# b41sh/pa

Measured on AMD Instinct MI355X. Metric: decoded GB/s (uncompressed) per node at 1/2/4/8 GPUs; bit-exact vs CPU, higher is better.
Workload: dtype int32

## Files before the change

### pa_amd/csrc/sb_decode.hip

```cpp
#include <hip/hip_runtime.h>
#include <stdint.h>

#include <algorithm>
#include <cstdlib>
#include <map>
#include <mutex>
#include <type_traits>

#include "sb_internal.h"

namespace sbk {

using namespace sb;

#ifndef SB_BLOCK
#define SB_BLOCK 256
#endif
#ifndef SB_LOAD_NT
#define SB_LOAD_NT 1
#endif
#ifndef SB_STORE_NT
#define SB_STORE_NT 1
#endif
#ifndef SB_LDS_DMA
// ... 3861 lines not shown
          run_leaf<1>(s, sh, rs, [&](uint32_t row, const uint32_t* v, uint32_t nv) {
            uint32_t nib = 0;
            for (uint32_t l = 0; l < nv; l++) nib |= (v[l] != 0 ? 1u : 0u) << l;
            if (nib) atomicOr(&xbits[row >> 5], nib << (row & 31));
          });
          __syncthreads();
          if (!sh.err) write_validity(xs, 0, n, pd.row_off, (uint32_t*)a.out_values);
          break;
        }
        case 1:
        case 3: {
          if (tid < 64) {
            const uint32_t r = expand_to_lds(st.codec, a.chunk + pd.byte_off + st.body, st.csize, (lds_u8*)xbits,
                                             (n + 7) / 8);
            if (r) set_err(sh, r);
          }
          __syncthreads();
          if (!sh.err) write_validity(xs, 0, n, pd.row_off, (uint32_t*)a.out_values);
          break;
        }
        case 2:
          if (!Z || need + xb + kZTablesBytes + kStagePad > a.stage_bytes) {
            if (tid == 0) set_err(sh, ST_NYI);
            break;
          }
          if constexpr (Z) if (tid < 64) {
            const uint32_t r = zs::zstd_to_lds(LdsSrc{s.w, s.base + st.body}, st.csize, (lds_u8*)xbits, (n + 7) / 8,
                                               (lds_u8*)xbits + xb, a.stage_bytes - need - xb - kStagePad);
            if (r) set_err(sh, r);
          }
          __syncthreads();
          if (!sh.err) write_validity(xs, 0, n, pd.row_off, (uint32_t*)a.out_values);
          break;
        default:
          if (tid == 0) set_err(sh, ST_OUT_OF_SPEC);
      }
    }
    __syncthreads();
    if (tid == 0) a.status[page] = sh.err;
    __syncthreads();
  }
}

constexpr uint32_t kLvK = 32;
constexpr uint32_t kMaxRuns = 64;

struct LvRuns {
  uint32_t n;
  uint32_t start[kMaxRuns + 1];
  uint32_t arg[kMaxRuns];
};

struct ListShared {
  uint32_t rows, vpos, bw_def, region, fast;
  LvRuns rep, def;
};

__device__ __forceinline__ void put_err(uint32_t* err, uint32_t code) { *err = max(*err, code); }

template <class Src>
__device__ bool parse_runs(const Src& s, uint32_t* err, uint32_t p, uint32_t end, uint32_t L, uint32_t bw, LvRuns& R) {
  uint32_t covered = 0, n = 0;
  while (covered < L) {
    uint32_t h = 0, sft = 0;
    for (;;) {
      if (p >= end || sft > 28) { put_err(err, ST_OUT_OF_SPEC); return false; }
      const uint32_t c = s.u8(p++);
      h |= (c & 0x7Fu) << sft;
      if (!(c & 0x80)) break;
      sft += 7;
    }
    if (n == kMaxRuns) { put_err(err, ST_NYI); return false; }
    R.start[n] = covered;
    if (h & 1) {
      const uint64_t want = (uint64_t)(h >> 1) * bw;
      const uint32_t have = (uint32_t)min<uint64_t>(want, end - p);
      const uint32_t vals = (uint32_t)min<uint64_t>((uint64_t)(h >> 1) * 8, (uint64_t)have * 8 / bw);
      if (vals == 0) { put_err(err, ST_OUT_OF_SPEC); return false; }
      R.arg[n] = 0x80000000u | p;
      p += have;
      covered += vals;
    } else {
      const uint32_t vb = (bw + 7) / 8;
      if (p + vb > end) { put_err(err, ST_OUT_OF_SPEC); return false; }
      uint32_t v = 0;
      for (uint32_t k = 0; k < vb; k++) v |= s.u8(p + k) << (8 * k);
      R.arg[n] = v;
      p += vb;
      covered += h >> 1;
    }
    n++;
  }
  R.start[n] = covered;
  R.n = n;
  return true;
}

template <class Src>
__device__ __forceinline__ uint32_t level_at(const Src& s, const LvRuns& R, uint32_t i, uint32_t bw) {
  uint32_t r = 0;
  if (R.n > 1) {
    uint32_t lo = 0, hi = R.n;
    while (hi - lo > 1) {
      const uint32_t mid = (lo + hi) >> 1;
      if (R.start[mid] <= i) lo = mid; else hi = mid;
    }
    r = lo;
  }
  const uint32_t a = R.arg[r];
  if (!(a & 0x80000000u)) return a;
  const uint32_t bit = (i - R.start[r]) * bw;
  return (s.u32((a & 0x7FFFFFFFu) + (bit >> 3)) >> (bit & 7)) & ((1u << bw) - 1);
}

struct ListArgs {
  const uint8_t* chunk;
  const PageDesc* pages;
  uint32_t n_pages;
  uint32_t nl, ni, ow;
  uint32_t width;
  uint32_t peek;
  uint64_t* counts;
  uint64_t* local;
  uint64_t* blk;
  uint64_t* totals;
  uint4* lvdesc;
  PageDesc* vpages;
  uint8_t* out_offsets;
  uint32_t* out_list_validity;
  uint32_t* out_leaf_validity;
  uint32_t* status;
  uint32_t epoch;
};

template <class Src>
__device__ bool list_parse(const Src& s, uint32_t* err, ListShared& ls, const PageDesc& pd, const ListArgs& a) {
  const uint32_t len = pd.byte_len, L = pd.num_values;
  if (len < 12) { put_err(err, ST_IO); return false; }
  const uint32_t rows = s.u32(0), rl = s.u32(4), dl = s.u32(8);
  if ((uint64_t)12 + rl + dl > len) { put_err(err, ST_IO); return false; }
  const uint32_t max_def = a.nl + 1 + a.ni;
  ls.rows = rows;
  ls.vpos = 12 + rl + dl;
  ls.region = 12 + rl + dl;
  ls.bw_def = 32 - __clz(max_def);
  if (!parse_runs(s, err, 12, 12 + rl, L, 1, ls.rep)) return false;
  if (!parse_runs(s, err, 12 + rl, 12 + rl + dl, L, ls.bw_def, ls.def)) return false;
  if (L > 0 && rows == 0) { put_err(err, ST_OUT_OF_SPEC); return false; }
  ls.fast = ls.rep.n == 1 && (ls.rep.arg[0] & 0x80000000u) && ls.def.n == 1 && (ls.def.arg[0] & 0x80000000u) &&
            ls.bw_def <= 2;
  return true;
}

__device__ __forceinline__ uint32_t compact_even(uint64_t x) {
  x &= 0x5555555555555555ull;
  x = (x | (x >> 1)) & 0x3333333333333333ull;
  x = (x | (x >> 2)) & 0x0F0F0F0F0F0F0F0Full;
  x = (x | (x >> 4)) & 0x00FF00FF00FF00FFull;
  x = (x | (x >> 8)) & 0x0000FFFF0000FFFFull;
  x = (x | (x >> 16)) & 0x00000000FFFFFFFFull;
  return (uint32_t)x;
}

template <class Src>
__device__ __forceinline__ uint64_t ld_bytes(const Src& s, uint32_t p, uint32_t nb, uint32_t end) {
  if (p + 8 <= end) return s.u64(p) & (nb >= 8 ? ~0ull : ((1ull << (8 * nb)) - 1));
  uint64_t v = 0;
  for (uint32_t k = 0; k < nb && p + k < end; k++) v |= (uint64_t)s.u8(p + k) << (8 * k);
  return v;
}

struct LvMasks {
  uint32_t vm, rsm, lfm, lvm, fvm;
};

template <class Src>
__device__ __forceinline__ LvMasks fast_level_masks(const Src& s, uint32_t rp, uint32_t dp, uint32_t region, uint32_t bw,
                                                    uint32_t i0, uint32_t L, uint32_t cs1) {
  LvMasks m{0, 0, 0, 0, 0};
  if (i0 >= L) return m;
  m.vm = L - i0 >= 32 ? 0xFFFFFFFFu : ((1u << (L - i0)) - 1);
  const uint32_t repw = (uint32_t)ld_bytes(s, rp + i0 / 8, 4, dp);
  m.rsm = ~repw & m.vm;
  const uint64_t dw = ld_bytes(s, dp + i0 * bw / 8, 4 * bw, region);
  auto ge = [&](uint32_t t) -> uint32_t {
    if (t == 0) return 0xFFFFFFFFu;
    if (bw == 1) return t == 1 ? (uint32_t)dw : 0u;
    const uint32_t lo = compact_even(dw), hi = compact_even(dw >> 1);
    return t == 1 ? (lo | hi) : t == 2 ? hi : (hi & lo);
  };
  m.lfm = ge(cs1) & m.vm;
  m.lvm = ge(1) & m.vm;
  m.fvm = ge(cs1 + 1) & m.vm;
  return m;
}

template <class Src>
__device__ __forceinline__ LvMasks level_masks(const Src& s, const ListShared& ls, uint32_t i0, uint32_t L,
                                               uint32_t cs1) {
  if (ls.fast)
    return fast_level_masks(s, ls.rep.arg[0] & 0x7FFFFFFFu, ls.def.arg[0] & 0x7FFFFFFFu, ls.region, ls.bw_def, i0, L, cs1);
  LvMasks m{0, 0, 0, 0, 0};
  if (i0 >= L) return m;
  m.vm = L - i0 >= 32 ? 0xFFFFFFFFu : ((1u << (L - i0)) - 1);
  const uint32_t bw = ls.bw_def;
  for (uint32_t k = 0; k < 32; k++) {
    const uint32_t i = i0 + k;
    if (i >= L) break;
    const uint32_t r = level_at(s, ls.rep, i, 1), d = level_at(s, ls.def, i, bw);
    if (r == 0) m.rsm |= 1u << k;
    if (r <= 1 && d >= cs1) m.lfm |= 1u << k;
    if (d > 0) m.lvm |= 1u << k;
    if (d > cs1) m.fvm |= 1u << k;
  }
  return m;
}

__device__ __forceinline__ void lds_or_bits(uint32_t* bm, uint32_t pos, uint64_t v, uint32_t nbits) {
  if (!nbits || !v) return;
  const uint32_t w = pos >> 5, sft = pos & 31;
  const uint64_t lo = v << sft;
  atomicOr(&bm[w], (uint32_t)lo);
  if ((uint32_t)(lo >> 32)) atomicOr(&bm[w + 1], (uint32_t)(lo >> 32));
}

__device__ __forceinline__ void wave_sync() {
  __builtin_amdgcn_fence(__ATOMIC_ACQ_REL, "wavefront");
  __builtin_amdgcn_wave_barrier();
}


__device__ __forceinline__ void wave_put_bits(const uint32_t* bm, uint32_t n, uint64_t g0, uint32_t* out) {
  if (n == 0) return;
  const uint32_t sh = (uint32_t)(g0 & 31), nw = (sh + n + 31) >> 5, eb = (sh + n) & 31;
  uint32_t* o = out + (g0 >> 5);
  for (uint32_t i = threadIdx.x & 63; i < nw; i += 64) {
    const uint32_t v = sh ? __builtin_amdgcn_alignbit(bm[i], bm[(int)i - 1], 32 - sh) : bm[i];
    const bool lo_edge = i == 0 && sh, hi_edge = i == nw - 1 && eb;
    if (lo_edge || hi_edge) {
      uint32_t m = lo_edge ? ~0u << sh : ~0u;
      if (hi_edge) m &= (1u << eb) - 1;
      atomicAnd(&o[i], ~m);
      if (v) atomicOr(&o[i], v);
    } else {
      o[i] = v;
    }
  }
}

#ifndef SB_LV_STAGE
#define SB_LV_STAGE 4160
#endif
#ifndef SB_LV_STAGE_PAD
#define SB_LV_STAGE_PAD 16
#endif
constexpr uint32_t kLvStage = SB_LV_STAGE;
constexpr uint32_t kLvStep = 64 * kLvK;

#ifndef SB_LV_ACC_BITS
#define SB_LV_ACC_BITS 8192
#endif
constexpr uint32_t kLvAccBits = SB_LV_ACC_BITS;
constexpr uint32_t kLvBitsW = kLvAccBits / 32 + 2;

struct ListWave {
  ListShared ls;
  uint32_t err;
  alignas(16) uint16_t obuf[kLvStep + 8];
  uint32_t lbits[kLvBitsW];
  uint32_t fbits[kLvBitsW];
};

struct LvAcc {
  uint32_t r, l;
  uint64_t g0, v0;
};

struct StageSrc {
  LdsSrc l;
  GlbSrc g;
  uint32_t lim;
  __device__ __forceinline__ uint32_t u8(uint32_t i) const { return i < lim ? l.u8(i) : g.u8(i); }
  __device__ __forceinline__ uint32_t u32(uint32_t i) const { return i + 4 <= lim ? l.u32(i) : g.u32(i); }
  __device__ __forceinline__ uint64_t u64(uint32_t i) const { return i + 8 <= lim ? l.u64(i) : g.u64(i); }
};

__device__ __forceinline__ uint32_t compress32(uint32_t x, uint32_t m) {
  x &= m;
  uint32_t mk = ~m << 1;
#pragma unroll
  for (int i = 0; i < 5; i++) {
    uint32_t mp = mk ^ (mk << 1);
    mp ^= mp << 2;
    mp ^= mp << 4;
    mp ^= mp << 8;
    mp ^= mp << 16;
    const uint32_t mv = mp & m;
    m = (m ^ mv) | (mv >> (1 << i));
    const uint32_t t = x & mv;
    x = (x ^ t) | (t >> (1 << i));
    mk &= ~mp;
  }
  return x;
}

__device__ __forceinline__ void lv_flush(ListWave& w, const ListArgs& a, LvAcc& acc) {
  const uint32_t lane = threadIdx.x & 63;
#ifndef SB_V_LV_NOBITS
  if (a.nl) wave_put_bits(w.lbits + 1, acc.r, acc.g0, a.out_list_validity);
  if (a.ni) wave_put_bits(w.fbits + 1, acc.l, acc.v0, a.out_leaf_validity);
#endif
  wave_sync();
  const uint32_t nw = (max(acc.r, acc.l) + 31) / 32 + 2;
  for (uint32_t i = lane; i < nw; i += 64) w.lbits[i] = w.fbits[i] = 0;
  wave_sync();
  acc.g0 += acc.r;
  acc.v0 += acc.l;
  acc.r = acc.l = 0;
}

template <bool WRITE, class WV>
__device__ uint32_t lv_step_m(const LvMasks m, WV& w, uint32_t rows, const ListArgs& a, uint32_t t0, uint64_t rbase,
                              uint64_t lbase, uint32_t carry_r, uint32_t carry_l, uint32_t* step_r, uint32_t* step_l,
                              LvAcc& acc) {
  const uint32_t lane = threadIdx.x & 63;
  if (t0 == 0 && lane == 0 && !(m.rsm & 1)) put_err(&w.err, ST_OUT_OF_SPEC);
  const uint32_t pk = ((uint32_t)__popc(m.rsm) << 16) | (uint32_t)__popc(m.lfm);
  const uint32_t incl = wave_incl_scan(pk), tot = __builtin_amdgcn_readlane(incl, 63), ex = incl - pk;
  const uint32_t rb = carry_r + (ex >> 16), lb = carry_l + (ex & 0xFFFFu);
  uint32_t cm = m.vm;
  if (rb + __popc(m.rsm) > rows) {
    if (rb >= rows + 1) cm = 0;
    else {
      uint32_t x = m.rsm;
      for (uint32_t k = rows - rb; k; k--) x &= x - 1;
      cm = (x & (0u - x)) - 1;
    }
  }
  const uint32_t rsm = m.rsm & cm, lfm = m.lfm & cm;
  if constexpr (WRITE) {
    const uint32_t s_r0 = carry_r, s_l0 = carry_l;
    const uint64_t g0 = rbase + s_r0, v0 = lbase + s_l0;
    const uint32_t al = a.ow == 4 ? (uint32_t)(g0 & 3) : (uint32_t)(g0 & 1);
    if (acc.r + (tot >> 16) > kLvAccBits || acc.l + (tot & 0xFFFFu) > kLvAccBits) lv_flush(w, a, acc);
    const uint32_t pr = acc.r + rb - s_r0, pf = acc.l + lb - s_l0;
    const uint32_t nr = __popc(rsm), nf = __popc(lfm);
    uint16_t* ob = w.obuf + al + (rb - s_r0);
    const uint32_t lrel = lb - s_l0;
    uint32_t j = 0;
#ifndef SB_V_LV_NOOB
    for (uint32_t x = rsm; x; x &= x - 1, j++) ob[j] = (uint16_t)(lrel + __popc(m.lfm & ((x & (0u - x)) - 1)));
#endif
    if (a.nl) lds_or_bits(w.lbits + 1, pr, compress32(m.lvm, rsm), nr);
    if (a.ni) lds_or_bits(w.fbits + 1, pf, compress32(m.fvm, lfm), nf);
    const uint32_t cpk = (nr << 16) | nf;
    const uint32_t ctot = __builtin_amdgcn_readlane(wave_incl_scan(cpk), 63);
    const uint32_t tr = ctot >> 16, tl = ctot & 0xFFFFu;
    wave_sync();
#ifdef SB_V_LV_NOOFF
    constexpr bool wr_off = false;
#else
    constexpr bool wr_off = true;
#endif
    if (!wr_off) {
    } else if (a.ow == 4) {
      uint32_t* o = (uint32_t*)a.out_offsets + (g0 - al);
      const uint32_t v32 = (uint32_t)v0, nq = (al + tr + 3) >> 2;
      for (uint32_t q = lane; q < nq; q += 64) {
        const uint32_t* pr = (const uint32_t*)(w.obuf + 4 * q);
        const uint32_t px = pr[0], py = pr[1];
        const uint32_t e0 = v32 + (px & 0xFFFFu), e1 = v32 + (px >> 16), e2 = v32 + (py & 0xFFFFu), e3 = v32 + (py >> 16);
        const uint32_t j0 = 4 * q;
        if (j0 >= al && j0 + 4 <= al + tr) {
          st_out((u32x4*)(o + j0), u32x4{e0, e1, e2, e3});
        } else {
          const uint32_t e[4] = {e0, e1, e2, e3};
#pragma unroll
          for (uint32_t k = 0; k < 4; k++)
            if (j0 + k >= al && j0 + k < al + tr) o[j0 + k] = e[k];
        }
      }
    } else {
      uint64_t* o = (uint64_t*)a.out_offsets + (g0 - al);
      const uint32_t nq = (al + tr + 1) >> 1;
      for (uint32_t q = lane; q < nq; q += 64) {
        const uint32_t j0 = 2 * q;
        const uint64_t x0 = v0 + w.obuf[j0], x1 = v0 + w.obuf[j0 + 1];
        if (j0 >= al && j0 + 2 <= al + tr) {
          st_out((u32x4*)(o + j0), u32x4{(uint32_t)x0, (uint32_t)(x0 >> 32), (uint32_t)x1, (uint32_t)(x1 >> 32)});
        } else {
          if (j0 >= al && j0 < al + tr) o[j0] = x0;
          if (j0 + 1 >= al && j0 + 1 < al + tr) o[j0 + 1] = x1;
        }
      }
    }
    acc.r += tr;
    acc.l += tl;
    wave_sync();
  }
  *step_r = tot >> 16;
  *step_l = tot & 0xFFFFu;
  return __builtin_amdgcn_readlane(wave_incl_scan(__popc(lfm)), 63);
}

template <bool WRITE, class Src>
__device__ __forceinline__ uint32_t lv_step(const Src& s, ListWave& w, const ListShared& ls, const ListArgs& a,
                                            uint32_t t0, uint32_t L, uint64_t rbase, uint64_t lbase, uint32_t carry_r,
                                            uint32_t carry_l, uint32_t* step_r, uint32_t* step_l, LvAcc& acc) {
  const LvMasks m = level_masks(s, ls, t0 + (threadIdx.x & 63) * kLvK, L, a.nl + 1);
  return lv_step_m<WRITE>(m, w, ls.rows, a, t0, rbase, lbase, carry_r, carry_l, step_r, step_l, acc);
}

template <bool WRITE, class Src>
__device__ void wave_levels(const Src& s, ListWave& w, const ListArgs& a, uint32_t L, uint64_t rbase, uint64_t lbase,
                            uint32_t* rows_c, uint32_t* leaves_c) {
  const uint32_t lane = threadIdx.x & 63, rows = w.ls.rows;
  uint32_t carry_r = 0, carry_l = 0, leaves = 0;
  LvAcc acc{0, 0, rbase, lbase};
  if constexpr (WRITE) {
    for (uint32_t i = lane; i < kLvBitsW; i += 64) w.lbits[i] = w.fbits[i] = 0;
    wave_sync();
  }
  for (uint32_t t0 = 0; t0 < L; t0 += kLvStep) {
    uint32_t sr, sl;
    leaves += lv_step<WRITE>(s, w, w.ls, a, t0, L, rbase, lbase, carry_r, carry_l, &sr, &sl, acc);
    carry_r += sr;
    carry_l += sl;
    if (carry_r > rows) break;
  }
  if constexpr (WRITE) lv_flush(w, a, acc);
  const uint32_t rc = min(carry_r, rows);
  if (lane == 0 && rc != rows) put_err(&w.err, ST_OUT_OF_SPEC);
  *rows_c = rc;
  *leaves_c = leaves;
}

template <class Src>
__device__ __forceinline__ uint32_t lv_count(const Src& s, const ListShared& ls, uint32_t t0, uint32_t L, uint32_t cs1) {
  const LvMasks m = level_masks(s, ls, t0 + (threadIdx.x & 63) * kLvK, L, cs1);
  const uint32_t pk = ((uint32_t)__popc(m.rsm) << 16) | (uint32_t)__popc(m.lfm);
  return __builtin_amdgcn_readlane(wave_incl_scan(pk), 63);
}

__device__ bool wave_page_setup(ListWave& w, uint32_t* stage, const ListArgs& a, uint32_t page, const PageDesc& pd, bool reuse,
                                bool* staged, uint32_t* mis_out, uint32_t* lim_out) {
  const uint32_t lane = threadIdx.x & 63;
  const uint8_t* pg = a.chunk + pd.byte_off;
  const uintptr_t a0 = (uintptr_t)pg & ~(uintptr_t)3;
  const uint32_t mis = (uint32_t)((uintptr_t)pg & 3);
  const uint32_t lim = stage ? min(pd.byte_len, kLvStage) : 0u;
  const uint32_t ndw = (mis + lim + 3) >> 2;
  uint4 d0 = make_uint4(0, 0, 0, 0), d1 = d0;
  if (reuse) {
    d0 = a.lvdesc[2 * page];
    d1 = a.lvdesc[2 * page + 1];
  }
  if (stage) {
    typedef const __attribute__((address_space(1))) uint32_t g32;
    constexpr uint32_t kIt = (kLvStage / 4 + 2 + 63) / 64;
    uint32_t v[kIt];
#pragma unroll
    for (uint32_t k = 0; k < kIt; k++) {
      const uint32_t d = lane + 64 * k;
      v[k] = d < ndw ? __builtin_nontemporal_load((g32*)a0 + d) : 0u;
    }
#pragma unroll
    for (uint32_t k = 0; k < kIt; k++)
      if (lane + 64 * k < ndw) stage[lane + 64 * k] = v[k];
  }
  if (lane == 0) w.err = 0;
  wave_sync();
  *mis_out = mis;
  *lim_out = lim;
  if (reuse && (d0.w & 1)) {
    if (lane == 0) {
      w.ls.rows = d0.x;
      w.ls.vpos = d0.y;
      w.ls.region = d0.y;
      w.ls.bw_def = d0.w >> 1;
      w.ls.fast = 1;
      w.ls.rep.n = w.ls.def.n = 1;
      w.ls.rep.start[0] = w.ls.def.start[0] = 0;
      w.ls.rep.arg[0] = 0x80000000u | d0.z;
      w.ls.def.arg[0] = 0x80000000u | d1.x;
    }
  } else if (lane == 0) {
    const StageSrc ss{LdsSrc{stage, mis}, GlbSrc{pg}, lim};
    list_parse(ss, &w.err, w.ls, pd, a);
  }
  wave_sync();
  if (w.err) return false;
  *staged = w.ls.region <= lim;
  return true;
}

__global__ __launch_bounds__(NT) void k_list_size(ListArgs a) {
  __shared__ ListWave waves[NW];
  __shared__ uint32_t stages[NW][kLvStage / 4 + SB_LV_STAGE_PAD];
  const uint32_t lane = threadIdx.x & 63;
  ListWave& w = waves[threadIdx.x >> 6];
  uint32_t* stage = stages[threadIdx.x >> 6];
  for (uint32_t page = blockIdx.x * NW + (threadIdx.x >> 6); page < a.n_pages; page += gridDim.x * NW) {
    const PageDesc pd = a.pages[page];
    bool staged = false;
    uint32_t mis = 0, lim = 0, rows_c = 0, leaves_c = 0;
    if (wave_page_setup(w, stage, a, page, pd, false, &staged, &mis, &lim)) {
      if (staged) wave_levels<false>(LdsSrc{stage, mis}, w, a, pd.num_values, 0, 0, &rows_c, &leaves_c);
      else wave_levels<false>(GlbSrc{a.chunk + pd.byte_off}, w, a, pd.num_values, 0, 0, &rows_c, &leaves_c);
    }
    wave_sync();
    if (lane == 0) {
      const bool ok = w.err == 0;
      a.counts[page] = ok ? (((uint64_t)rows_c << 32) | leaves_c) : 0;
      const uint32_t fast = ok && w.ls.fast;
      a.lvdesc[2 * page] = make_uint4(w.ls.rows, w.ls.vpos, w.ls.rep.arg[0] & 0x7FFFFFFFu, fast | (w.ls.bw_def << 1));
      a.lvdesc[2 * page + 1] = make_uint4(w.ls.def.arg[0] & 0x7FFFFFFFu, ok, 0, 0);
      a.status[page] = w.err;
    }
    wave_sync();
  }
}

__global__ __launch_bounds__(NT) void k_list_bscan(ListArgs a) {
  __shared__ Shared sh;
  const uint32_t p = blockIdx.x * NT + threadIdx.x;
  uint64_t c = 0;
  if (p < a.n_pages) {
    if (a.peek) {
      const PageDesc pd = a.pages[p];
      const GlbSrc g{a.chunk + pd.byte_off};
      if (pd.byte_len >= 12) {
        const uint64_t vpos = 12ull + g.u32(4) + g.u32(8);
        if (vpos + 9 <= pd.byte_len) c = ((uint64_t)g.u32(0) << 32) | (g.u32((uint32_t)vpos + 5) / a.width);
      }
      a.counts[p] = c;
    } else {
      c = a.counts[p];
    }
  }
  uint64_t tr, tl;
  const uint64_t er = block_excl_scan<uint64_t>(c >> 32, sh, &tr);
  const uint64_t el = block_excl_scan<uint64_t>(c & 0xFFFFFFFFull, sh, &tl);
  if (p < a.n_pages) {
    a.local[2 * p] = er;
    a.local[2 * p + 1] = el;
  }
  if (threadIdx.x == 0) {
    a.blk[2 * blockIdx.x] = tr;
    a.blk[2 * blockIdx.x + 1] = tl;
  }
}

__global__ __launch_bounds__(NT) void k_list_bases(ListArgs a) {
  __shared__ Shared sh;
  __shared__ uint64_t red[2][NW];
  const uint32_t tid = threadIdx.x, lane = tid & 63, wv = tid >> 6;
  const uint32_t p = blockIdx.x * NT + tid;
  uint64_t c = 0;
  uint64_t vpos = ~0ull;
  PageDesc pd{};
  if (p < a.n_pages) {
    if (a.peek) {
      pd = a.pages[p];
      const GlbSrc g{a.chunk + pd.byte_off};
      if (pd.byte_len >= 12) {
        vpos = 12ull + g.u32(4) + g.u32(8);
        if (vpos + 9 <= pd.byte_len) c = ((uint64_t)g.u32(0) << 32) | (g.u32((uint32_t)vpos + 5) / a.width);
      }
      a.counts[p] = c;
    } else {
      c = a.counts[p];
    }
  }
  uint64_t tr, tl;
  const uint64_t er = block_excl_scan<uint64_t>(c >> 32, sh, &tr);
  const uint64_t el = block_excl_scan<uint64_t>(c & 0xFFFFFFFFull, sh, &tl);
  constexpr uint64_t kVal = (1ull << 48) - 1;
  const uint64_t tag = (uint64_t)a.epoch << 48;
  if (tid == 0) {
    __hip_atomic_store(&a.blk[2 * blockIdx.x], tag | tr, __ATOMIC_RELAXED, __HIP_MEMORY_SCOPE_AGENT);
    __hip_atomic_store(&a.blk[2 * blockIdx.x + 1], tag | tl, __ATOMIC_RELAXED, __HIP_MEMORY_SCOPE_AGENT);
  }
  if (wv == 0) {
    uint64_t br = 0, bl = 0;
    for (uint32_t b0 = 0; b0 < blockIdx.x; b0 += 64) {
      const uint32_t b = b0 + lane;
      const bool need = b < blockIdx.x;
      uint64_t r = 0, l = 0;
      for (;;) {
        if (need) {
          r = __hip_atomic_load(&a.blk[2 * b], __ATOMIC_RELAXED, __HIP_MEMORY_SCOPE_AGENT);
          l = __hip_atomic_load(&a.blk[2 * b + 1], __ATOMIC_RELAXED, __HIP_MEMORY_SCOPE_AGENT);
        }
        if (!__ballot(need && ((r & ~kVal) != tag || (l & ~kVal) != tag))) break;
        __builtin_amdgcn_s_sleep(1);
      }
      if (need) {
        br += r & kVal;
        bl += l & kVal;
      }
    }
    br = wave_sum64(br);
    bl = wave_sum64(bl);
    if (lane == 0) {
      red[0][0] = br;
      red[1][0] = bl;
    }
  }
  __syncthreads();
  if (p < a.n_pages) {
    const uint64_t rbase = red[0][0] + er, lbase = red[1][0] + el;
    a.local[2 * p] = rbase;
    a.local[2 * p + 1] = lbase;
    if (p == a.n_pages - 1) {
      const uint64_t tr_all = rbase + (c >> 32), tl_all = lbase + (c & 0xFFFFFFFFull);
      if (a.nl && a.out_list_validity && (tr_all & 31)) a.out_list_validity[tr_all >> 5] = 0;
      if (a.ni && a.out_leaf_validity && (tl_all & 31)) a.out_leaf_validity[tl_all >> 5] = 0;
    }
    if (a.peek) {
      const bool ok = vpos + 9 <= pd.byte_len;
      a.vpages[p] = PageDesc{pd.byte_off + (ok ? vpos : 0), lbase, ok ? pd.byte_len - (uint32_t)vpos : 0,
                             ok ? (uint32_t)c : 0, a.vpages[p].reserved};
    }
  }
}

__global__ __launch_bounds__(NT) void k_list_levels(ListArgs a) {
  __shared__ ListWave waves[NW];
  __shared__ uint32_t stages[NW][kLvStage / 4 + SB_LV_STAGE_PAD];
  const uint32_t lane = threadIdx.x & 63;
  ListWave& w = waves[threadIdx.x >> 6];
  uint32_t* stage = stages[threadIdx.x >> 6];
  for (uint32_t page = blockIdx.x * NW + (threadIdx.x >> 6); page < a.n_pages; page += gridDim.x * NW) {
    const PageDesc pd = a.pages[page];
    const uint64_t rbase = a.local[2 * page], lbase = a.local[2 * page + 1];
    const uint64_t cnt = a.counts[page];
    bool staged = false;
    uint32_t mis = 0, lim = 0, rows_c = 0, leaves_c = 0;
    const bool sized = a.lvdesc[2 * page + 1].y != 0;
    if (sized && wave_page_setup(w, stage, a, page, pd, true, &staged, &mis, &lim)) {
      if (staged) wave_levels<true>(LdsSrc{stage, mis}, w, a, pd.num_values, rbase, lbase, &rows_c, &leaves_c);
      else wave_levels<true>(GlbSrc{a.chunk + pd.byte_off}, w, a, pd.num_values, rbase, lbase, &rows_c, &leaves_c);
    } else if (lane == 0) {
      w.err = 0;
      if (!sized) {
        const StageSrc ss{LdsSrc{nullptr, 0}, GlbSrc{a.chunk + pd.byte_off}, 0};
        list_parse(ss, &w.err, w.ls, pd, a);
        if (!w.err) w.err = ST_OUT_OF_SPEC;
      }
    }
    wave_sync();
    if (lane == 0) {
      uint32_t err = w.err;
      if (!err && (rows_c != (uint32_t)(cnt >> 32) || leaves_c != (uint32_t)cnt)) err = ST_OUT_OF_SPEC;
      const bool ok = err == 0;
      if (!a.peek)
        a.vpages[page] = PageDesc{pd.byte_off + (ok ? w.ls.vpos : 0), lbase, ok ? pd.byte_len - w.ls.vpos : 0,
                                  ok ? leaves_c : 0, a.vpages[page].reserved};
      a.status[page] = err;
      if (page == a.n_pages - 1) {
        const uint64_t tr = rbase + (cnt >> 32), tl = lbase + (uint32_t)cnt;
        a.totals[0] = tr;
        a.totals[1] = tl;
        if (a.out_offsets) bin_put_off(a.out_offsets, tr, tl, a.ow);
      }
    }
    wave_sync();
  }
}

struct NestArgs {
  const uint8_t* chunk;
  const PageDesc* pages;
  uint32_t n_pages, depth, nullable, ow, smask;
  uint64_t* counts;
  const uint64_t* bases;
  const uint64_t* totals;
  PageDesc* vpages;
  uint8_t* out_offsets[kMaxNest];
  uint32_t* out_validity[kMaxNest];
  uint32_t* out_leaf_validity;
  uint32_t* status;
  uint32_t* vpos;
};

struct RunWin {
  uint32_t n, p, end, covered, bw;
  uint32_t start[68];
  uint32_t arg[68];
};

__device__ bool runwin_advance(const GlbSrc& s, RunWin& R, uint32_t l0, uint32_t lend, uint32_t* err) {
  if (R.bw == 0) {
    R.n = 1;
    R.start[0] = 0;
    R.arg[0] = 0;
    R.covered = 0xFFFFFFFFu;
    R.start[1] = R.covered;
    return true;
  }
  uint32_t k = R.n;
  while (k > 0 && R.start[k - 1] > l0) k--;
  if (k > 1) {
    for (uint32_t i = k - 1; i < R.n; i++) {
      R.start[i - (k - 1)] = R.start[i];
      R.arg[i - (k - 1)] = R.arg[i];
    }
    R.n -= k - 1;
  }
  while (R.covered < lend) {
    if (R.n >= 66) { put_err(err, ST_NYI); return false; }
    uint32_t h = 0, sft = 0;
    for (;;) {
      if (R.p >= R.end || sft > 28) { put_err(err, ST_OUT_OF_SPEC); return false; }
      const uint32_t c = s.u8(R.p++);
      h |= (c & 0x7Fu) << sft;
      if (!(c & 0x80)) break;
      sft += 7;
    }
    uint32_t cnt, arg;
    if (h & 1) {
      const uint64_t want = (uint64_t)(h >> 1) * R.bw;
      const uint32_t have = (uint32_t)min<uint64_t>(want, R.end - R.p);
      cnt = (uint32_t)min<uint64_t>((uint64_t)(h >> 1) * 8, (uint64_t)have * 8 / max(R.bw, 1u));
      arg = 0x80000000u | R.p;
      R.p += have;
    } else {
      const uint32_t vb = (R.bw + 7) / 8;
      if (R.p + vb > R.end) { put_err(err, ST_OUT_OF_SPEC); return false; }
      arg = 0;
      for (uint32_t b = 0; b < vb; b++) arg |= s.u8(R.p + b) << (8 * b);
      R.p += vb;
      cnt = h >> 1;
    }
    if (cnt == 0) continue;
    R.start[R.n] = R.covered;
    R.arg[R.n] = arg;
    R.n++;
    R.covered += cnt;
  }
  R.start[R.n] = R.covered;
  return true;
}

__device__ __forceinline__ uint32_t runwin_at(const GlbSrc& s, const RunWin& R, uint32_t i) {
  uint32_t lo = 0, hi = R.n;
  while (hi - lo > 1) {
    const uint32_t mid = (lo + hi) >> 1;
    if (R.start[mid] <= i) lo = mid; else hi = mid;
  }
  const uint32_t a = R.arg[lo];
  if (!(a & 0x80000000u)) return a;
  const uint32_t bit = (i - R.start[lo]) * R.bw;
  return (s.u32((a & 0x7FFFFFFFu) + (bit >> 3)) >> (bit & 7)) & ((1u << R.bw) - 1);
}

struct NestWave {
  RunWin rep, def;
  uint32_t err, rows, vpos;
};

__device__ __forceinline__ uint64_t compress64(uint64_t v, uint64_t m) {
  const uint32_t lo = compress32((uint32_t)v, (uint32_t)m), hi = compress32((uint32_t)(v >> 32), (uint32_t)(m >> 32));
  return (uint64_t)lo | ((uint64_t)hi << __popc((uint32_t)m));
}

__device__ __forceinline__ void put_bits64(uint32_t* bm, uint64_t pos, uint64_t v, uint32_t n) {
  const uint32_t lane = threadIdx.x & 63;
  if (!n || !v || lane > 2) return;
  const uint32_t sh = (uint32_t)(pos & 31);
  const uint64_t w0 = pos >> 5;
  const uint32_t word = lane == 0 ? (uint32_t)(v << sh)
                      : lane == 1 ? (uint32_t)(sh ? (v >> (32 - sh)) : (v >> 32))
                                  : (uint32_t)(sh ? (v >> (64 - sh)) : 0u);
  if (word) atomicOr(&bm[w0 + lane], word);
}

template <bool WRITE>
__global__ __launch_bounds__(NT) void k_nest_walk(NestArgs a) {
  __shared__ NestWave waves[NW];
  const uint32_t lane = threadIdx.x & 63, D = a.depth;
  NestWave& w = waves[threadIdx.x >> 6];
  uint32_t cum_sum[kMaxNest + 2], cum_rep[kMaxNest + 2];
  cum_sum[0] = cum_rep[0] = 0;
  for (uint32_t d = 0; d <= D; d++) {
    const uint32_t nl = (a.nullable >> d) & 1, rp = (d < D && !((a.smask >> d) & 1)) ? 1u : 0u;
    cum_sum[d + 1] = cum_sum[d] + nl + rp;
    cum_rep[d + 1] = cum_rep[d] + rp;
  }
  const uint64_t below = lane ? (~0ull >> (64 - lane)) : 0ull;
  for (uint32_t page = blockIdx.x * NW + (threadIdx.x >> 6); page < a.n_pages; page += gridDim.x * NW) {
    const PageDesc pd = a.pages[page];
    const GlbSrc s{a.chunk + pd.byte_off};
    const uint32_t L = pd.num_values;
    if (lane == 0) {
      w.err = 0;
      const uint32_t len = pd.byte_len;
      if (len < 12) {
        w.err = ST_IO;
      } else {
        const uint32_t rows = s.u32(0), rl = s.u32(4), dl = s.u32(8);
        if ((uint64_t)12 + rl + dl > len) {
          w.err = ST_IO;
        } else {
          w.rows = rows;
          w.vpos = 12 + rl + dl;
          w.rep = RunWin{0, 12, 12 + rl, 0, 32u - __clz(cum_rep[D + 1])};
          w.def = RunWin{0, 12 + rl, 12 + rl + dl, 0, 32u - __clz(cum_sum[D + 1])};
          if (L > 0 && rows == 0) w.err = ST_OUT_OF_SPEC;
        }
      }
    }
    wave_sync();
    uint64_t carry[kMaxNest + 1] = {0, 0, 0, 0, 0}, base[kMaxNest + 1] = {0, 0, 0, 0, 0};
    if (WRITE)
      for (uint32_t d = 0; d <= D; d++) base[d] = a.bases[(uint64_t)page * (D + 1) + d];
    uint32_t rows_seen = 0;
    const uint32_t rows = w.rows;
    if (!w.err) {
      for (uint32_t l0 = 0; l0 < L; l0 += 64) {
// ... 107 lines not shown
  const uint32_t lds = L.lds_bytes ? std::min(L.lds_bytes, kDeferredLds) : kDeferredLds;
  sbk::BinArgs a{L.chunk, L.pages, L.n_pages, L.nullable, L.sizes, L.bases, L.total, L.out_offsets, L.out_values,
                 L.values_cap, L.out_validity, L.status, lds, L.jobs, L.job_count, L.scratch, L.lds_need, L.cls,
                 L.region, L.rneed, L.lb, L.checked};
  hipStream_t st = (hipStream_t)stream;
  const dim3 block(sbk::NT);
  const dim3 grid(std::max<uint32_t>(1, L.staged_grid));
  const dim3 cgrid((L.n_pages + sbk::NT - 1) / sbk::NT);
  const dim3 lgrid(std::min<uint32_t>(L.n_pages, 65535u));
  const dim3 bgrid(std::max<uint32_t>(1, std::min<uint32_t>(L.n_big, 1024u)));
  ensure_lds_attr(sbk::k_bin_size<4, true>, (int)kDeferredLds);
  ensure_lds_attr(sbk::k_bin_size<8, true>, (int)kDeferredLds);
  ensure_lds_attr(sbk::k_bin_decode<4, true>, (int)kDeferredLds);
  ensure_lds_attr(sbk::k_bin_decode<8, true>, (int)kDeferredLds);
  ensure_lds_attr(sbk::k_bin_fused<4, true>, (int)kDeferredLds);
  ensure_lds_attr(sbk::k_bin_fused<8, true>, (int)kDeferredLds);
  ensure_lds_attr(sbk::k_bin_size<4, false>, (int)kDeferredLds);
  ensure_lds_attr(sbk::k_bin_size<8, false>, (int)kDeferredLds);
  ensure_lds_attr(sbk::k_bin_decode<4, false>, (int)kDeferredLds);
  ensure_lds_attr(sbk::k_bin_decode<8, false>, (int)kDeferredLds);
  ensure_lds_attr(sbk::k_bin_fused<4, false>, (int)kDeferredLds);
  ensure_lds_attr(sbk::k_bin_fused<8, false>, (int)kDeferredLds);
  const bool z = L.zstd != 0;
  if (stage == 2) {
    if (offset_width == 8) hipLaunchKernelGGL(sbk::k_bin_probe<8>, cgrid, block, 0, st, a);
    else hipLaunchKernelGGL(sbk::k_bin_probe<4>, cgrid, block, 0, st, a);
  } else if (stage == 0) {
    if (hipMemsetAsync(L.cls + 4 * (size_t)L.n_pages, 0, 3 * sizeof(uint32_t), st) != hipSuccess) return -1;
    if (offset_width == 8) {
      hipLaunchKernelGGL(sbk::k_bin_light<8>, cgrid, block, 0, st, a);
      if (z) hipLaunchKernelGGL((sbk::k_bin_size<8, true>), grid, block, lds, st, a);
      else hipLaunchKernelGGL((sbk::k_bin_size<8, false>), grid, block, lds, st, a);
      if (L.n_big) hipLaunchKernelGGL((sbk::k_bin_big<8, 0>), bgrid, block, sbk::kBigLds, st, a);
    } else {
      hipLaunchKernelGGL(sbk::k_bin_light<4>, cgrid, block, 0, st, a);
      if (z) hipLaunchKernelGGL((sbk::k_bin_size<4, true>), grid, block, lds, st, a);
      else hipLaunchKernelGGL((sbk::k_bin_size<4, false>), grid, block, lds, st, a);
      if (L.n_big) hipLaunchKernelGGL((sbk::k_bin_big<4, 0>), bgrid, block, sbk::kBigLds, st, a);
    }
    hipLaunchKernelGGL(sbk::k_bin_scan, dim3(1), block, 0, st, a);
  } else if (stage == 3) {
    if (hipMemsetAsync(L.lb, 0, (L.n_pages + 1) * sizeof(uint64_t), st) != hipSuccess) return -1;
    if (offset_width == 8) {
      if (z) hipLaunchKernelGGL((sbk::k_bin_fused<8, true>), grid, block, lds, st, a);
      else hipLaunchKernelGGL((sbk::k_bin_fused<8, false>), grid, block, lds, st, a);
    } else {
      if (z) hipLaunchKernelGGL((sbk::k_bin_fused<4, true>), grid, block, lds, st, a);
      else hipLaunchKernelGGL((sbk::k_bin_fused<4, false>), grid, block, lds, st, a);
    }
  } else {
    if (offset_width == 8) {
      if (z) hipLaunchKernelGGL((sbk::k_bin_decode<8, true>), grid, block, lds, st, a);
      else hipLaunchKernelGGL((sbk::k_bin_decode<8, false>), grid, block, lds, st, a);
      if (L.n_big) hipLaunchKernelGGL((sbk::k_bin_big<8, 1>), bgrid, block, sbk::kBigLds, st, a);
      hipLaunchKernelGGL(sbk::k_bin_light_out<8>, lgrid, block, 0, st, a);
    } else {
      if (z) hipLaunchKernelGGL((sbk::k_bin_decode<4, true>), grid, block, lds, st, a);
      else hipLaunchKernelGGL((sbk::k_bin_decode<4, false>), grid, block, lds, st, a);
      if (L.n_big) hipLaunchKernelGGL((sbk::k_bin_big<4, 1>), bgrid, block, sbk::kBigLds, st, a);
      hipLaunchKernelGGL(sbk::k_bin_light_out<4>, lgrid, block, 0, st, a);
    }
  }
  return hipGetLastError() == hipSuccess ? 0 : -1;
}
int launch_utf8_check(int offset_width, const Utf8Launch& a, void* stream) {
  if (a.n_rows == 0 || a.n_pages == 0) return 0;
  hipStream_t st = (hipStream_t)stream;
  const uint64_t chunks = (a.len + 15) / 16;
  if (chunks && a.ascii) {
    const dim3 g(std::min<uint32_t>(a.n_pages, 65535u));
    if ((uintptr_t)a.values % 16) hipLaunchKernelGGL(sbk::k_utf8_pages<false>, g, dim3(sbk::NT), 0, st, a);
    else hipLaunchKernelGGL(sbk::k_utf8_pages<true>, g, dim3(sbk::NT), 0, st, a);
  } else if (chunks) {
    const dim3 g((uint32_t)std::max<uint64_t>(1, std::min<uint64_t>((chunks + sbk::NT - 1) / sbk::NT, 8192)));
    if ((uintptr_t)a.values % 16) hipLaunchKernelGGL(sbk::k_utf8_bytes<false>, g, dim3(sbk::NT), 0, st, a);
    else hipLaunchKernelGGL(sbk::k_utf8_bytes<true>, g, dim3(sbk::NT), 0, st, a);
  }
  const dim3 g((uint32_t)std::min<uint64_t>((a.n_rows + sbk::NT) / sbk::NT, 8192));
  if (offset_width == 8) hipLaunchKernelGGL(sbk::k_utf8_bounds<8>, g, dim3(sbk::NT), 0, st, a);
  else hipLaunchKernelGGL(sbk::k_utf8_bounds<4>, g, dim3(sbk::NT), 0, st, a);
  return hipGetLastError() == hipSuccess ? 0 : -1;
}
}

#ifdef SB_INF_PHASES
extern "C" int sb_debug_inf_phases(uint64_t* host) {
  return hipMemcpyFromSymbol(host, HIP_SYMBOL(sbk::sb_dbg_inf), 16 * 8) == hipSuccess ? 0 : -1;
}
extern "C" int sb_debug_inf_reset() {
  static const unsigned long long z[16] = {0};
  return hipMemcpyToSymbol(HIP_SYMBOL(sbk::sb_dbg_inf), z, sizeof z) == hipSuccess ? 0 : -1;
}
#endif
#ifdef SB_BIN_PHASES
extern "C" int sb_debug_bin_phases(uint64_t* host, uint64_t n) {
  return hipMemcpyFromSymbol(host, HIP_SYMBOL(sbk::sb_dbg_phase), std::min<uint64_t>(n, 4096 * 6) * 8) == hipSuccess ? 0 : -1;
}
#endif

namespace sb {
static uint32_t inflate_resident() {
  static std::mutex mu;
  static std::map<int, uint32_t> cache;
  int dev = 0;
  (void)hipGetDevice(&dev);
  std::lock_guard<std::mutex> g(mu);
  auto it = cache.find(dev);
  if (it != cache.end()) return it->second;
  int per_cu = 0, cus = 0;
  if (hipOccupancyMaxActiveBlocksPerMultiprocessor(&per_cu, (const void*)sbk::k_inflate, 64 * sbk::kInfWaves, 0) !=
          hipSuccess ||
      hipDeviceGetAttribute(&cus, hipDeviceAttributeMultiprocessorCount, dev) != hipSuccess || per_cu <= 0 || cus <= 0)
    per_cu = 0;
  const uint32_t r = per_cu ? (uint32_t)(std::min(per_cu, SB_INF_BLOCKS) * cus) : kInflateGrid;
  cache[dev] = r;
  return r;
}
extern "C" uint32_t sb_debug_inflate_resident() { return inflate_resident(); }
int launch_inflate(const InflateLaunch& a, void* stream) {
  if (a.n_jobs == 0) return 0;
  if (a.patas_wg && launch_patas(a, stream))
    return -1;
  static const bool stat = getenv("SB_INF_STATIC") != nullptr;
  static const uint32_t gcap = getenv("SB_INF_GRID") ? (uint32_t)atoi(getenv("SB_INF_GRID")) : 0u;
  InflateLaunch b = a;
  if (stat) b.sched = nullptr;
  uint32_t cap = b.sched ? std::min<uint32_t>(inflate_resident(), kInflateGrid) : kInflateGrid;
  if (gcap) cap = gcap;
  const uint32_t grid = std::min<uint32_t>((a.n_jobs + sbk::kInfWaves - 1) / sbk::kInfWaves, cap);
  hipLaunchKernelGGL(sbk::k_inflate, dim3(grid), dim3(64 * sbk::kInfWaves), 0, (hipStream_t)stream, b);
  return hipGetLastError() == hipSuccess ? 0 : -1;
}
int launch_zinflate(const InflateLaunch& a, void* stream) {
  if (a.n_jobs == 0) return 0;
  const uint32_t grid = std::min<uint32_t>(a.n_jobs, 1024u);
  hipLaunchKernelGGL(sbk::k_zinflate, dim3(grid), dim3(64), 0, (hipStream_t)stream, a);
  return hipGetLastError() == hipSuccess ? 0 : -1;
}
}

namespace sb {
int launch_bool(const LaunchArgs& a, void* stream) {
  if (a.n_list == 0) return 0;
  ensure_lds_attr(sbk::k_bool_decode<true>, (int)kDeferredLds);
  ensure_lds_attr(sbk::k_bool_decode<false>, (int)kDeferredLds);
  const uint32_t grid = std::min<uint32_t>(a.n_list, 65535u);
  if (a.zstd) hipLaunchKernelGGL(sbk::k_bool_decode<true>, dim3(grid), dim3(sbk::NT), a.stage_bytes, (hipStream_t)stream, a);
  else hipLaunchKernelGGL(sbk::k_bool_decode<false>, dim3(grid), dim3(sbk::NT), a.stage_bytes, (hipStream_t)stream, a);
  return hipGetLastError() == hipSuccess ? 0 : -1;
}
}

namespace sb {
int launch_list(int stage, const ListLaunch& L, void* stream) {
  sbk::ListArgs a{L.chunk, L.pages, L.n_pages, L.list_nullable, L.item_nullable, L.offset_width, L.width, L.peek,
                  L.counts, L.local, L.blk, L.totals, (uint4*)L.lvdesc, L.vpages, L.out_offsets, L.out_list_validity,
                  L.out_leaf_validity, L.status, L.epoch};
  if (L.n_pages == 0) return 0;
  const uint32_t grid = std::min<uint32_t>((L.n_pages + sbk::NW - 1) / sbk::NW, kListGrid);
  const uint32_t nblk = (L.n_pages + sbk::NT - 1) / sbk::NT;
  hipStream_t st = (hipStream_t)stream;
  if (stage == 0) {
    hipLaunchKernelGGL(sbk::k_list_size, dim3(grid), dim3(sbk::NT), 0, st, a);
  } else if (stage == 1) {
    hipLaunchKernelGGL(sbk::k_list_bscan, dim3(nblk), dim3(sbk::NT), 0, st, a);
  } else if (stage == 4) {
    hipLaunchKernelGGL(sbk::k_list_bases, dim3(nblk), dim3(sbk::NT), 0, st, a);
  } else {
    hipLaunchKernelGGL(sbk::k_list_levels, dim3(grid), dim3(sbk::NT), 0, st, a);
  }
  return hipGetLastError() == hipSuccess ? 0 : -1;
}
}

namespace sb {
int launch_nest(int stage, const NestLaunch& L, void* stream) {
  if (L.n_pages == 0) return 0;
  sbk::NestArgs a{L.chunk, L.pages, L.n_pages, L.depth, L.nullable, L.offset_width, L.struct_mask, L.counts, L.bases, L.totals,
                  L.vpages, {}, {}, L.out_leaf_validity, L.status, L.vpos};
  for (int d = 0; d < kMaxNest; d++) {
    a.out_offsets[d] = L.out_offsets[d];
    a.out_validity[d] = L.out_validity[d];
  }
  const uint32_t grid = std::min<uint32_t>((L.n_pages + sbk::NW - 1) / sbk::NW, kListGrid);
  if (stage == 0) hipLaunchKernelGGL(sbk::k_nest_walk<false>, dim3(grid), dim3(sbk::NT), 0, (hipStream_t)stream, a);
  else hipLaunchKernelGGL(sbk::k_nest_walk<true>, dim3(grid), dim3(sbk::NT), 0, (hipStream_t)stream, a);
  return hipGetLastError() == hipSuccess ? 0 : -1;
}
}
```

Measured before the change: 4442.

## Prefetch next list page into registers and add fast paths in level decoding

The list levels kernel now software-pipelines its page loop: each wave loads the next page's bytes into registers while it processes the current staged page, and it prefetches page descriptors two iterations ahead. The goal is to hide global load latency. Several smaller changes come with it. A cheaper 32-bit bit-unzip replaces the 64-bit compact_even. A wave-uniform no-cut flag skips the row-cut logic and a redundant scan. A ballot skips compress32 when all values are valid. The block size and grid are now set by a configurable waves-per-block constant and by an occupancy query. Keeping the prefetch in registers raises register pressure, which may lower occupancy.

```diff
diff --git a/pa_amd/csrc/sb_decode.hip b/pa_amd/csrc/sb_decode.hip
--- a/pa_amd/csrc/sb_decode.hip
+++ b/pa_amd/csrc/sb_decode.hip
@@ -4037,14 +4037,13 @@
   return true;
 }
 
-__device__ __forceinline__ uint32_t compact_even(uint64_t x) {
-  x &= 0x5555555555555555ull;
-  x = (x | (x >> 1)) & 0x3333333333333333ull;
-  x = (x | (x >> 2)) & 0x0F0F0F0F0F0F0F0Full;
-  x = (x | (x >> 4)) & 0x00FF00FF00FF00FFull;
-  x = (x | (x >> 8)) & 0x0000FFFF0000FFFFull;
-  x = (x | (x >> 16)) & 0x00000000FFFFFFFFull;
-  return (uint32_t)x;
+__device__ __forceinline__ uint32_t unzip16(uint32_t w) {
+  uint32_t t;
+  t = (w ^ (w >> 1)) & 0x22222222u; w ^= t ^ (t << 1);
+  t = (w ^ (w >> 2)) & 0x0C0C0C0Cu; w ^= t ^ (t << 2);
+  t = (w ^ (w >> 4)) & 0x00F000F0u; w ^= t ^ (t << 4);
+  t = (w ^ (w >> 8)) & 0x0000FF00u; w ^= t ^ (t << 8);
+  return w;
 }
 
 template <class Src>
@@ -4068,12 +4067,13 @@
   const uint32_t repw = (uint32_t)ld_bytes(s, rp + i0 / 8, 4, dp);
   m.rsm = ~repw & m.vm;
   const uint64_t dw = ld_bytes(s, dp + i0 * bw / 8, 4 * bw, region);
-  auto ge = [&](uint32_t t) -> uint32_t {
-    if (t == 0) return 0xFFFFFFFFu;
-    if (bw == 1) return t == 1 ? (uint32_t)dw : 0u;
-    const uint32_t lo = compact_even(dw), hi = compact_even(dw >> 1);
-    return t == 1 ? (lo | hi) : t == 2 ? hi : (hi & lo);
-  };
+  uint32_t lo = (uint32_t)dw, hi = 0;
+  if (bw == 2) {
+    const uint32_t u0 = unzip16((uint32_t)dw), u1 = unzip16((uint32_t)(dw >> 32));
+    lo = (u0 & 0xFFFFu) | (u1 << 16);
+    hi = (u0 >> 16) | (u1 & 0xFFFF0000u);
+  }
+  auto ge = [&](uint32_t t) -> uint32_t { return t == 0 ? 0xFFFFFFFFu : t == 1 ? (lo | hi) : t == 2 ? hi : (hi & lo); };
   m.lfm = ge(cs1) & m.vm;
   m.lvm = ge(1) & m.vm;
   m.fvm = ge(cs1 + 1) & m.vm;
@@ -4141,6 +4141,10 @@
 #endif
 constexpr uint32_t kLvStage = SB_LV_STAGE;
 constexpr uint32_t kLvStep = 64 * kLvK;
+#ifndef SB_LV_NW
+#define SB_LV_NW 4
+#endif
+constexpr uint32_t kLvNW = SB_LV_NW;
 
 #ifndef SB_LV_ACC_BITS
 #define SB_LV_ACC_BITS 8192
@@ -4187,6 +4191,11 @@
     mk &= ~mp;
   }
   return x;
+}
+
+__device__ __forceinline__ uint32_t compress_valid(uint32_t x, uint32_t m, uint32_t n) {
+  if (!__ballot((x & m) != m)) return (uint32_t)((1ull << n) - 1);
+  return compress32(x, m);
 }
 
 __device__ __forceinline__ void lv_flush(ListWave& w, const ListArgs& a, LvAcc& acc) {
@@ -4213,8 +4222,9 @@
   const uint32_t pk = ((uint32_t)__popc(m.rsm) << 16) | (uint32_t)__popc(m.lfm);
   const uint32_t incl = wave_incl_scan(pk), tot = __builtin_amdgcn_readlane(incl, 63), ex = incl - pk;
   const uint32_t rb = carry_r + (ex >> 16), lb = carry_l + (ex & 0xFFFFu);
+  const bool nocut = __builtin_amdgcn_readfirstlane(carry_r) + (tot >> 16) <= __builtin_amdgcn_readfirstlane(rows);
   uint32_t cm = m.vm;
-  if (rb + __popc(m.rsm) > rows) {
+  if (!nocut && rb + __popc(m.rsm) > rows) {
     if (rb >= rows + 1) cm = 0;
     else {
       uint32_t x = m.rsm;
@@ -4223,6 +4233,7 @@
     }
   }
   const uint32_t rsm = m.rsm & cm, lfm = m.lfm & cm;
+  uint32_t consumed = 0;
   if constexpr (WRITE) {
     const uint32_t s_r0 = carry_r, s_l0 = carry_l;
     const uint64_t g0 = rbase + s_r0, v0 = lbase + s_l0;
@@ -4236,11 +4247,11 @@
 #ifndef SB_V_LV_NOOB
     for (uint32_t x = rsm; x; x &= x - 1, j++) ob[j] = (uint16_t)(lrel + __popc(m.lfm & ((x & (0u - x)) - 1)));
 #endif
-    if (a.nl) lds_or_bits(w.lbits + 1, pr, compress32(m.lvm, rsm), nr);
-    if (a.ni) lds_or_bits(w.fbits + 1, pf, compress32(m.fvm, lfm), nf);
-    const uint32_t cpk = (nr << 16) | nf;
-    const uint32_t ctot = __builtin_amdgcn_readlane(wave_incl_scan(cpk), 63);
+    if (a.nl) lds_or_bits(w.lbits + 1, pr, compress_valid(m.lvm, rsm, nr), nr);
+    if (a.ni) lds_or_bits(w.fbits + 1, pf, compress_valid(m.fvm, lfm, nf), nf);
+    const uint32_t ctot = nocut ? tot : __builtin_amdgcn_readlane(wave_incl_scan((nr << 16) | nf), 63);
     const uint32_t tr = ctot >> 16, tl = ctot & 0xFFFFu;
+    consumed = tl;
     wave_sync();
 #ifdef SB_V_LV_NOOFF
     constexpr bool wr_off = false;
@@ -4285,7 +4296,8 @@
   }
   *step_r = tot >> 16;
   *step_l = tot & 0xFFFFu;
-  return __builtin_amdgcn_readlane(wave_incl_scan(__popc(lfm)), 63);
+  if constexpr (!WRITE) consumed = nocut ? tot & 0xFFFFu : __builtin_amdgcn_readlane(wave_incl_scan(__popc(lfm)), 63);
+  return consumed;
 }
 
 template <bool WRITE, class Src>
@@ -4327,32 +4339,37 @@
   return __builtin_amdgcn_readlane(wave_incl_scan(pk), 63);
 }
 
-__device__ bool wave_page_setup(ListWave& w, uint32_t* stage, const ListArgs& a, uint32_t page, const PageDesc& pd, bool reuse,
-                                bool* staged, uint32_t* mis_out, uint32_t* lim_out) {
+constexpr uint32_t kLvStageIt = (kLvStage / 4 + 2 + 63) / 64;
+
+__device__ __forceinline__ uint32_t lv_stage_dwords(const ListArgs& a, const PageDesc& pd) {
+  return ((uint32_t)((uintptr_t)(a.chunk + pd.byte_off) & 3) + min(pd.byte_len, kLvStage) + 3) >> 2;
+}
+
+__device__ __forceinline__ void lv_stage_load(const ListArgs& a, const PageDesc& pd, uint32_t (&v)[kLvStageIt]) {
+  typedef const __attribute__((address_space(1))) uint32_t g32;
+  const uint32_t lane = threadIdx.x & 63, ndw = lv_stage_dwords(a, pd);
+  const uintptr_t a0 = (uintptr_t)(a.chunk + pd.byte_off) & ~(uintptr_t)3;
+#pragma unroll
+  for (uint32_t k = 0; k < kLvStageIt; k++) {
+    const uint32_t d = lane + 64 * k;
+    v[k] = d < ndw ? __builtin_nontemporal_load((g32*)a0 + d) : 0u;
+  }
+}
+
+__device__ __forceinline__ void lv_stage_store(uint32_t* stage, const ListArgs& a, const PageDesc& pd,
+                                               const uint32_t (&v)[kLvStageIt]) {
+  const uint32_t lane = threadIdx.x & 63, ndw = lv_stage_dwords(a, pd);
+#pragma unroll
+  for (uint32_t k = 0; k < kLvStageIt; k++)
+    if (lane + 64 * k < ndw) stage[lane + 64 * k] = v[k];
+}
+
+__device__ bool wave_page_parse(ListWave& w, uint32_t* stage, const ListArgs& a, const PageDesc& pd, bool reuse, uint4 d0,
+                                uint4 d1, bool* staged, uint32_t* mis_out, uint32_t* lim_out) {
   const uint32_t lane = threadIdx.x & 63;
   const uint8_t* pg = a.chunk + pd.byte_off;
-  const uintptr_t a0 = (uintptr_t)pg & ~(uintptr_t)3;
   const uint32_t mis = (uint32_t)((uintptr_t)pg & 3);
-  const uint32_t lim = stage ? min(pd.byte_len, kLvStage) : 0u;
-  const uint32_t ndw = (mis + lim + 3) >> 2;
-  uint4 d0 = make_uint4(0, 0, 0, 0), d1 = d0;
-  if (reuse) {
-    d0 = a.lvdesc[2 * page];
-    d1 = a.lvdesc[2 * page + 1];
-  }
-  if (stage) {
-    typedef const __attribute__((address_space(1))) uint32_t g32;
-    constexpr uint32_t kIt = (kLvStage / 4 + 2 + 63) / 64;
-    uint32_t v[kIt];
-#pragma unroll
-    for (uint32_t k = 0; k < kIt; k++) {
-      const uint32_t d = lane + 64 * k;
-      v[k] = d < ndw ? __builtin_nontemporal_load((g32*)a0 + d) : 0u;
-    }
-#pragma unroll
-    for (uint32_t k = 0; k < kIt; k++)
-      if (lane + 64 * k < ndw) stage[lane + 64 * k] = v[k];
-  }
+  const uint32_t lim = min(pd.byte_len, kLvStage);
   if (lane == 0) w.err = 0;
   wave_sync();
   *mis_out = mis;
@@ -4389,7 +4406,10 @@
     const PageDesc pd = a.pages[page];
     bool staged = false;
     uint32_t mis = 0, lim = 0, rows_c = 0, leaves_c = 0;
-    if (wave_page_setup(w, stage, a, page, pd, false, &staged, &mis, &lim)) {
+    uint32_t sv[kLvStageIt];
+    lv_stage_load(a, pd, sv);
+    lv_stage_store(stage, a, pd, sv);
+    if (wave_page_parse(w, stage, a, pd, false, make_uint4(0, 0, 0, 0), make_uint4(0, 0, 0, 0), &staged, &mis, &lim)) {
       if (staged) wave_levels<false>(LdsSrc{stage, mis}, w, a, pd.num_values, 0, 0, &rows_c, &leaves_c);
       else wave_levels<false>(GlbSrc{a.chunk + pd.byte_off}, w, a, pd.num_values, 0, 0, &rows_c, &leaves_c);
     }
@@ -4510,20 +4530,43 @@
   }
 }
 
-__global__ __launch_bounds__(NT) void k_list_levels(ListArgs a) {
-  __shared__ ListWave waves[NW];
-  __shared__ uint32_t stages[NW][kLvStage / 4 + SB_LV_STAGE_PAD];
-  const uint32_t lane = threadIdx.x & 63;
-  ListWave& w = waves[threadIdx.x >> 6];
-  uint32_t* stage = stages[threadIdx.x >> 6];
-  for (uint32_t page = blockIdx.x * NW + (threadIdx.x >> 6); page < a.n_pages; page += gridDim.x * NW) {
-    const PageDesc pd = a.pages[page];
-    const uint64_t rbase = a.local[2 * page], lbase = a.local[2 * page + 1];
-    const uint64_t cnt = a.counts[page];
+struct LvPage {
+  PageDesc pd;
+  uint64_t rbase, lbase, cnt;
+  uint4 d0, d1;
+};
+
+__device__ __forceinline__ LvPage lv_page(const ListArgs& a, uint32_t page) {
+  return LvPage{a.pages[page], a.local[2 * page], a.local[2 * page + 1], a.counts[page], a.lvdesc[2 * page],
+                a.lvdesc[2 * page + 1]};
+}
+
+__global__ __launch_bounds__(64 * kLvNW) void k_list_levels(ListArgs a) {
+  __shared__ ListWave waves[kLvNW];
+  __shared__ uint32_t stages[kLvNW][kLvStage / 4 + SB_LV_STAGE_PAD];
+  const uint32_t lane = threadIdx.x & 63, wv = __builtin_amdgcn_readfirstlane(threadIdx.x >> 6);
+  ListWave& w = waves[wv];
+  uint32_t* stage = stages[wv];
+  const uint32_t stride = gridDim.x * kLvNW;
+  uint32_t page = blockIdx.x * kLvNW + wv;
+  if (page >= a.n_pages) return;
+  LvPage cur = lv_page(a, page);
+  LvPage nxt = page + stride < a.n_pages ? lv_page(a, page + stride) : cur;
+  uint32_t sv[kLvStageIt];
+  lv_stage_load(a, cur.pd, sv);
+  for (;;) {
+    const PageDesc pd = cur.pd;
+    const uint64_t rbase = cur.rbase, lbase = cur.lbase, cnt = cur.cnt;
+    lv_stage_store(stage, a, pd, sv);
+    const uint32_t np = page + stride;
+    const bool more = np < a.n_pages;
+    LvPage nn = nxt;
+    if (more && np + stride < a.n_pages) nn = lv_page(a, np + stride);
+    if (more) lv_stage_load(a, nxt.pd, sv);
     bool staged = false;
     uint32_t mis = 0, lim = 0, rows_c = 0, leaves_c = 0;
-    const bool sized = a.lvdesc[2 * page + 1].y != 0;
-    if (sized && wave_page_setup(w, stage, a, page, pd, true, &staged, &mis, &lim)) {
+    const bool sized = cur.d1.y != 0;
+    if (sized && wave_page_parse(w, stage, a, pd, true, cur.d0, cur.d1, &staged, &mis, &lim)) {
       if (staged) wave_levels<true>(LdsSrc{stage, mis}, w, a, pd.num_values, rbase, lbase, &rows_c, &leaves_c);
       else wave_levels<true>(GlbSrc{a.chunk + pd.byte_off}, w, a, pd.num_values, rbase, lbase, &rows_c, &leaves_c);
     } else if (lane == 0) {
@@ -4551,6 +4594,10 @@
       }
     }
     wave_sync();
+    if (!more) break;
+    page = np;
+    cur = nxt;
+    nxt = nn;
   }
 }
 
@@ -4964,6 +5011,23 @@
 }
 
 namespace sb {
+static uint32_t levels_resident() {
+  static std::mutex mu;
+  static std::map<int, uint32_t> cache;
+  int dev = 0;
+  (void)hipGetDevice(&dev);
+  std::lock_guard<std::mutex> g(mu);
+  auto it = cache.find(dev);
+  if (it != cache.end()) return it->second;
+  int per_cu = 0, cus = 0;
+  if (hipOccupancyMaxActiveBlocksPerMultiprocessor(&per_cu, (const void*)sbk::k_list_levels, 64 * sbk::kLvNW, 0) !=
+          hipSuccess ||
+      hipDeviceGetAttribute(&cus, hipDeviceAttributeMultiprocessorCount, dev) != hipSuccess || per_cu <= 0 || cus <= 0)
+    per_cu = 0;
+  const uint32_t r = per_cu ? (uint32_t)(per_cu * cus) : kListGrid * sbk::NW / sbk::kLvNW;
+  cache[dev] = r;
+  return r;
+}
 int launch_list(int stage, const ListLaunch& L, void* stream) {
   sbk::ListArgs a{L.chunk, L.pages, L.n_pages, L.list_nullable, L.item_nullable, L.offset_width, L.width, L.peek,
                   L.counts, L.local, L.blk, L.totals, (uint4*)L.lvdesc, L.vpages, L.out_offsets, L.out_list_validity,
@@ -4979,7 +5043,10 @@
   } else if (stage == 4) {
     hipLaunchKernelGGL(sbk::k_list_bases, dim3(nblk), dim3(sbk::NT), 0, st, a);
   } else {
-    hipLaunchKernelGGL(sbk::k_list_levels, dim3(grid), dim3(sbk::NT), 0, st, a);
+    static const uint32_t gcap = getenv("SB_LV_GRID") ? (uint32_t)atoi(getenv("SB_LV_GRID")) : 0u;
+    const uint32_t cap = gcap ? gcap : std::min<uint32_t>(levels_resident(), kListGrid * sbk::NW / sbk::kLvNW);
+    const uint32_t lgrid = std::min<uint32_t>((L.n_pages + sbk::kLvNW - 1) / sbk::kLvNW, cap);
+    hipLaunchKernelGGL(sbk::k_list_levels, dim3(lgrid), dim3(64 * sbk::kLvNW), 0, st, a);
   }
   return hipGetLastError() == hipSuccess ? 0 : -1;
 }
```

After: 4443, median of 3. No clear change (+0.0%).
